# Amandaynzhou/MMT-PSM

Measured on AMD Instinct MI355X. Metric: imgs/sec (student+teacher step, 1000x1000, AUG_K=2), higher is better.
Workload: dtype f32

## Files before the change

include/mmtpsm.h:

```cpp
#ifndef MMTPSM_H
#define MMTPSM_H
#include <stdint.h>
#ifdef __cplusplus
extern "C" {
#endif

#define MMT_EINVAL (-22)

int mmt_version(void);

typedef struct {
  const float* feat[4];
  float* grad_feat[4];
  int H[4];
  int W[4];
  float scale[4];
  int num_levels;
  int N;
  int C;
} mmt_pyramid;

int mmt_roi_align_forward(const mmt_pyramid* pyr , const float* rois, const int32_t* levels,
                          int K, int PH, int PW, int sampling_ratio, float* out, void* stream);
int mmt_roi_align_forward_bf16(const mmt_pyramid* pyr , const float* rois, const int32_t* levels,
// ... 106 lines not shown
  const void* w_src_scale;
  int x_planes_layout;
  void* y_rb;
  long y_rb_stride;
  const float* y_rb_scale;
  void* y_amax_next;
  int x_planes_lag;
  int y_rb_rows;
} mmt_conv_args;

int mmt_conv_forward(const mmt_conv_args* a , void* stream);
int mmt_conv_variant(const mmt_conv_args* a );
int mmt_conv_ksplit(const mmt_conv_args* a );
int mmt_conv_wants_planes(const mmt_conv_args* a );
int mmt_set_conv_precision(int mode);
int mmt_amax(const float* x, long n, const float* rowscale, long inner, int rows, float* amax , void* stream);
int mmt_amax_stats(const float* x, long n, float* slot , void* stream);
int mmt_sum_stats(const float* a, const float* b, const float* c, const float* d, float* y, long n,
                  float* slot , void* stream);
int mmt_stats_combine(const float* const* slots , int n, float* out , void* stream);
int mmt_split_planes_f16(const float* x, void* planes, long plane_stride, long n, float scale, const float* amax ,
                         float* scale_out , float* amax_next ,
                         float* zero_slot , void* stream);
int mmt_pack_weight_f16(const float* w, void* planes, long plane_stride, int Cout, int K, float scale, const float* amax,
                        float* scale_out, void* stream);
int mmt_pack_weight_flipped_f16(const float* w, const float* scale, void* planes, long plane_stride, int Cout, int KH, int KW,
                                int Cin, const float* amax, float* scale_out, void* stream);
int mmt_conv3x3_strip_f16x2(const mmt_conv_args* a , const float* s_x , const float* s_w , void* stream);
int mmt_conv_forward_f16x2(const mmt_conv_args* a , const float* x_amax , const float* s_w , void* stream);
int mmt_get_conv_precision(void);
int mmt_stem_fused(const float* x, int N, int H, int W, const float* w_s2d, const void* w_planes, long w_plane_stride,
                   const float* s_w , const float* scale, const float* shift, const float* x_slot , float* y,
                   float* y_slot , void* stream);
int mmt_conv_wgrad_planes_splits(const mmt_conv_args* a );
int mmt_conv_wgrad_planes(const mmt_conv_args* a , const float* dy, const void* x_planes, long x_plane_stride,
                          const void* dy_planes, long dy_plane_stride, const float* s_x, const float* s_dy, const float* rowscale,
                          float* dw, float* dbias, float* workspace, void* stream);
typedef struct {
  void* fn;
  long a[16];
} mmt_call;
int mmt_replay(const mmt_call* calls , int n, int* failed_index );
int mmt_split_planes_f16_rb(const float* x, void* planes, long plane_stride, int rows, int W, int C, const float* amax,
                            float* scale_out, void* stream);
int mmt_conv_writes_rb(const mmt_conv_args* a );
typedef struct mmt_wgrad_job {
  mmt_conv_args a;
  const float* dy; const float* rowscale; float* dw; float* dbias;
  const void* x_planes; long x_plane_stride; const void* dy_planes; long dy_plane_stride; const float* s_x; const float* s_dy;
} mmt_wgrad_job;
int mmt_conv_wgrad_group_workspace(const mmt_wgrad_job* jobs , int n, long* floats_out );
int mmt_conv_wgrad_group(const mmt_wgrad_job* jobs , int n, float* workspace, long workspace_floats, void* stream);
int mmt_sum_stats_rb(const float* a, const float* b, const float* c, const float* d, float* y, int rows, int W, int C, float* slot,
                     void* planes, long plane_stride, const float* scale, float* amax_next, void* stream);
int mmt_rb_scales_update(float* state, int n, void* stream);
int mmt_conv_forward_pg(const mmt_conv_args* a , const float* s_x , const float* s_w , int tile_rows,
                        int ksplit, void* stream);
int mmt_conv_pg_plan(const mmt_conv_args* a , int* tile_rows, int* ksplit);
int mmt_conv_pg_wanted(const mmt_conv_args* a );
typedef struct { long src_off, dst_off; int Cout, K, unit0, pad; } mmt_pack_desc;
long mmt_packed_weight_elems(int Cout, int K);
int mmt_pack_weight(const float* w, void* planes, long plane_stride, int Cout, int K, void* stream);
int mmt_pack_weight_flipped(const float* w, const float* scale, void* planes, long plane_stride, int Cout, int KH, int KW,
                            int Cin, void* stream);
int mmt_split_planes(const float* x, void* planes, long plane_stride, long n, void* stream);
typedef struct { const float* w; const float* scale; void* dst; long plane_stride; int Cout, KH, KW, Cin, unit0, pad; } mmt_flip_desc;
// ... 72 lines not shown
```

mmt-psm_amd/maskrcnn_benchmark/_hip.py:

```python
import ctypes
import weakref
import os
import threading as _threading

import torch

_HERE = os.path.dirname(os.path.abspath(__file__))
LIB_PATH = os.path.join(os.path.dirname(_HERE), "libmmtpsm.so")

c_void_p, c_int, c_float, c_double, c_int64 = ctypes.c_void_p, ctypes.c_int, ctypes.c_float, ctypes.c_double, ctypes.c_int64


class Pyramid(ctypes.Structure):
    _fields_ = [("feat", c_void_p * 4), ("grad_feat", c_void_p * 4), ("H", c_int * 4), ("W", c_int * 4),
                ("scale", c_float * 4), ("num_levels", c_int), ("N", c_int), ("C", c_int)]


class ConvArgs(ctypes.Structure):
    _fields_ = [("x", c_void_p), ("w", c_void_p), ("scale", c_void_p), ("shift", c_void_p), ("res", c_void_p),
                ("mask", c_void_p), ("mul", c_void_p), ("y", c_void_p),
                ("N", c_int), ("H", c_int), ("W", c_int), ("Cin", c_int), ("Cout", c_int), ("KH", c_int),
                ("KW", c_int), ("stride", c_int), ("pad", c_int), ("Ho", c_int), ("Wo", c_int),
                ("relu", c_int), ("res_mode", c_int), ("out_stride", c_int), ("out_H", c_int), ("out_W", c_int),
                ("mask_scale", c_float), ("w_planes", c_void_p), ("w_plane_stride", ctypes.c_long),
                ("x_planes", c_void_p), ("x_plane_stride", ctypes.c_long),
                ("y_planes", c_void_p), ("y_plane_stride", ctypes.c_long), ("io_bf16", c_int), ("y_amax", c_void_p),
                ("f16_x_amax", c_void_p), ("f16_dy_amax", c_void_p), ("y_amax_stats", c_int),
                ("f16_guard_x", c_void_p), ("f16_guard_dy", c_void_p), ("w_src", c_void_p), ("w_src_scale", c_void_p),
                ("x_planes_layout", c_int),
                ("y_rb", c_void_p), ("y_rb_stride", ctypes.c_long), ("y_rb_scale", c_void_p), ("y_amax_next", c_void_p),
                ("x_planes_lag", c_int), ("y_rb_rows", c_int)]


IO_X, IO_Y, IO_RES, IO_MASK, IO_DY = 1, 2, 4, 8, 16


class WgradJob(ctypes.Structure):
    _fields_ = [("a", ConvArgs), ("dy", c_void_p), ("rowscale", c_void_p), ("dw", c_void_p), ("dbias", c_void_p),
                ("x_planes", c_void_p), ("x_plane_stride", ctypes.c_long), ("dy_planes", c_void_p), ("dy_plane_stride", ctypes.c_long),
                ("s_x", c_void_p), ("s_dy", c_void_p)]


class RpnLevel(ctypes.Structure):
    _fields_ = [("head", c_void_p), ("anchors", c_void_p), ("topk", c_void_p), ("HW", c_int), ("k", c_int),
                ("out_off", c_int), ("pad", c_int)]


class RpnTopkLevel(ctypes.Structure):
    _fields_ = [("head", c_void_p), ("topk", c_void_p), ("HW", c_int), ("k", c_int)]


class RpnSelectArgs(ctypes.Structure):
    _fields_ = [("lv", RpnLevel * 8), ("L", c_int), ("N", c_int), ("A", c_int), ("C", c_int), ("sumk", c_int),
                ("clipv", c_float), ("lim", c_void_p), ("boxes", c_void_p), ("scores", c_void_p), ("idx", c_void_p),
                ("box_reg", c_void_p)]


class RpnPostArgs(ctypes.Structure):
    _fields_ = [("boxes", c_void_p), ("scores", c_void_p), ("idx", c_void_p), ("box_reg", c_void_p), ("keep", c_void_p),
                ("keep_cnt", c_void_p), ("seg_off", c_int * 9), ("own_pre", c_int * 8), ("L", c_int), ("N", c_int),
                ("sumk", c_int), ("kmax", c_int), ("post_n", c_int), ("fpn_post_n", c_int), ("training", c_int),
                ("cap", c_int), ("min_size_filter", c_int), ("pad", c_int), ("gt", c_void_p), ("gt_off", c_void_p),
                ("out_boxes", c_void_p), ("out_scores", c_void_p),
                ("out_idx", c_void_p), ("out_reg", c_void_p), ("out_level", c_void_p), ("out_cnt", c_void_p),
                ("key_scratch", c_void_p)]


# ... 57 lines not shown
                     c_void_p, c_void_p],
    "mmt_box_loss": [c_void_p, c_void_p, c_void_p, c_void_p, c_int, c_int, c_void_p, c_void_p, c_void_p, c_void_p],
    "mmt_box_loss_rows": [c_void_p, c_void_p, c_void_p, c_void_p, c_int, c_int, c_void_p, c_void_p, c_void_p, c_void_p, c_void_p],
    "mmt_relation_attention_fwd": [c_void_p, c_void_p, c_void_p, c_void_p, c_void_p, c_int, c_int, c_int, c_int, c_int, c_int, c_float,
                                   c_void_p, c_void_p, c_void_p],
    "mmt_relation_attention_bwd": [c_void_p, c_void_p, c_void_p, c_void_p, c_void_p, c_void_p, c_int, c_int, c_int, c_int, c_int, c_float,
                                   c_void_p, c_void_p, c_void_p, c_void_p, c_void_p, c_void_p],
    "mmt_ciam_fwd": [c_void_p, c_void_p, c_int, c_int, c_int, c_int, c_void_p, c_void_p, c_void_p, c_void_p, c_void_p],
    "mmt_ciam_bwd": [c_void_p, c_void_p, c_int, c_int, c_int, c_int, c_void_p, c_void_p, c_void_p, c_void_p, c_void_p, c_void_p,
                     c_void_p, c_void_p, c_void_p],
    "mmt_stats_combine": [c_void_p, c_int, c_void_p, c_void_p],
    "mmt_sum_stats": [c_void_p, c_void_p, c_void_p, c_void_p, c_void_p, ctypes.c_long, c_void_p, c_void_p],
    "mmt_split_planes_f16": [c_void_p, c_void_p, ctypes.c_long, ctypes.c_long, c_float, c_void_p, c_void_p, c_void_p, c_void_p, c_void_p],
    "mmt_split_planes_f16_rb": [c_void_p, c_void_p, ctypes.c_long, c_int, c_int, c_int, c_void_p, c_void_p, c_void_p],
    "mmt_replay": [c_void_p, c_int, c_void_p],
    "mmt_conv_writes_rb": [ctypes.POINTER(ConvArgs)],
    "mmt_conv_wgrad_group_workspace": [c_void_p, c_int, ctypes.POINTER(ctypes.c_long)],
    "mmt_conv_wgrad_group": [c_void_p, c_int, c_void_p, ctypes.c_long, c_void_p],
    "mmt_sum_stats_rb": [c_void_p, c_void_p, c_void_p, c_void_p, c_void_p, c_int, c_int, c_int, c_void_p, c_void_p, ctypes.c_long, c_void_p,
                         c_void_p, c_void_p],
    "mmt_rb_scales_update": [c_void_p, c_int, c_void_p],
    "mmt_conv_wgrad_planes_splits": [ctypes.POINTER(ConvArgs)],
    "mmt_conv_wgrad_planes": [ctypes.POINTER(ConvArgs), c_void_p, c_void_p, ctypes.c_long, c_void_p, ctypes.c_long, c_void_p, c_void_p,
                              c_void_p, c_void_p, c_void_p, c_void_p, c_void_p],
    "mmt_pack_weight_f16": [c_void_p, c_void_p, ctypes.c_long, c_int, c_int, c_float, c_void_p, c_void_p, c_void_p],
    "mmt_pack_weight_flipped_f16": [c_void_p, c_void_p, c_void_p, ctypes.c_long, c_int, c_int, c_int, c_int, c_void_p, c_void_p, c_void_p],
    "mmt_conv3x3_strip_f16x2": [ctypes.POINTER(ConvArgs), c_void_p, c_void_p, c_void_p],
    "mmt_conv_forward_f16x2": [ctypes.POINTER(ConvArgs), c_void_p, c_void_p, c_void_p],
    "mmt_conv_forward_pg": [ctypes.POINTER(ConvArgs), c_void_p, c_void_p, c_int, c_int, c_void_p],
    "mmt_conv_pg_plan": [ctypes.POINTER(ConvArgs), c_void_p, c_void_p],
    "mmt_conv_pg_wanted": [ctypes.POINTER(ConvArgs)],
    "mmt_stem_fused": [c_void_p, c_int, c_int, c_int, c_void_p, c_void_p, ctypes.c_long, c_void_p, c_void_p, c_void_p, c_void_p, c_void_p,
                       c_void_p, c_void_p],
    "mmt_maxpool3x3s2_bf16": [c_void_p, c_void_p, c_int, c_int, c_int, c_int, c_int, c_int, c_void_p],
    "mmt_gconv3x3_forward": [c_void_p, c_void_p, c_void_p, c_void_p, c_void_p, c_int, c_int, c_int, c_int, c_int, c_int, c_int, c_void_p],
    "mmt_gconv3x3_dgrad": [c_void_p, c_void_p, c_void_p, c_void_p, c_void_p, c_void_p, c_int, c_int, c_int, c_int, c_int, c_int, c_void_p],
    "mmt_gconv3x3_wgrad": [c_void_p, c_void_p, c_void_p, c_void_p, c_int, c_int, c_int, c_int, c_int, c_int, c_void_p],
    "mmt_mask_bce": [c_void_p, c_void_p, c_void_p, c_int, c_int, c_int, c_float, c_void_p, c_void_p, c_void_p],
    "mmt_mgd_level_forward": [c_void_p, ctypes.POINTER(MgdTeachers), c_void_p, c_int, c_int, c_int, c_int, c_void_p, c_void_p],
    "mmt_mgd_level_backward": [c_void_p, ctypes.POINTER(MgdTeachers), c_void_p, c_int, c_int, c_int, c_int, c_void_p, c_void_p, c_void_p],
    "mmt_mgd_views_forward": [ctypes.POINTER(MgdStudents), ctypes.POINTER(MgdTeachers), c_void_p, c_int, c_int, c_int, c_int, c_void_p,
                              c_void_p],
    "mmt_mgd_views_backward": [ctypes.POINTER(MgdStudents), ctypes.POINTER(MgdTeachers), c_void_p, c_int, c_int, c_int, c_int, c_void_p,
                               c_void_p, c_void_p],
    "mmt_mask_pool": [c_void_p, c_int, c_int, c_int, c_int, c_int, c_void_p, c_void_p],
    "mmt_psm_rows": [c_void_p, c_int, c_void_p, c_int, c_int, c_void_p, c_float, c_int, c_int, c_void_p, c_void_p, c_void_p],
    "mmt_psm_variance": [c_void_p, c_int, c_int, c_int, c_int, c_void_p, c_void_p],
    "mmt_ema_update": [c_void_p, c_void_p, c_int64, c_double, c_void_p],
    "mmt_sgd_momentum": [c_void_p, c_void_p, c_void_p, c_int64, c_float, c_float, c_float, c_int, c_void_p],
    "mmt_paste_masks": [c_void_p, c_void_p, c_void_p, c_void_p, c_int, c_int, c_int, c_int, c_int, c_float, c_void_p, c_void_p],
    "mmt_paste_mask_stack": [c_void_p, c_void_p, c_int, c_int, c_int, c_int, c_float, c_void_p, c_void_p],
    "mmt_polygon_targets": [c_void_p, c_void_p, c_void_p, c_void_p, c_int, c_int, c_void_p, c_void_p, c_void_p],
}

_lib = None
PROFILE = None
PROFILE_ALL = False
_BF16_STORAGE = os.environ.get("MMT_BF16_STORAGE", "0") != "0"


F16X2_DEFAULT = os.environ.get("MMT_F16X2", "1") != "0"
F16X2 = F16X2_DEFAULT
F16X2_TILED = True
F16_STATS = {"wgrad": 0, "conv": 0, "tiled": 0, "pg": 0, "amax_pass": 0, "fallback": 0, "weight_pack": 0}
WGRAD_F16_MIN_ELEMS = 1 << 22
_F16W = {}


def set_f16x2(on):
    global F16X2
    F16X2 = F16X2_DEFAULT if on is None else bool(on)
    _PLAN_EPOCH[0] += 1
    _PLAN.clear()
    _F16W.clear()
    _F16SITE.clear()
    _SITES.clear()
    rb_reset()


STAT_W = 40
_POOL_SLOTS = 2048
F16_CREST_HI, F16_CREST_LO = 2.0 ** 17, 2.0 ** 15


class _StatPool(object):
    __slots__ = ("dev", "host", "event", "next", "gen", "host_gen", "base")

    def __init__(self, device):
        self.dev = torch.zeros((_POOL_SLOTS, STAT_W), dtype=torch.float32, device=device)
        self.host = torch.zeros((_POOL_SLOTS, STAT_W), dtype=torch.float32).pin_memory()
        self.event, self.next, self.gen, self.host_gen = None, 0, 0, -1
        self.base = self.dev.data_ptr()

    def retire(self):
        self.host.copy_(self.dev, non_blocking=True)
        self.event = torch.cuda.Event()
        self.event.record()
# ... 527 lines not shown
    def __del__(self):
        try:
            p = self.pool
            if p is not None:
                self.pool = None
                _POOL_GRAVE.append(p)
        except Exception:
            pass


_POOL_GRAVE = []


def _drain_pools():
    while _POOL_GRAVE:
        try:
            _POOL_GRAVE.pop()
        except IndexError:
            break


def record_torch(fn):
    rec = getattr(_TLS, "rec", None)
    if rec is not None:
        def w(_fn=fn):
            _fn()
            return 0
        rec.calls.append((w, ()))


def planned(tag, fn, x):
    env = os.environ.get
    key = (tag, tuple(x.shape), x.dtype, _stream(), _PLAN_EPOCH[0], PLANES_EPOCH, LAYOUT_EPOCH[0], F16X2, _PREC, _BF16_STORAGE, _RB_EPOCH[0],
           env("MMT_STRIP"), env("MMT_SPLITK"), env("MMT_ROWS"), env("MMT_PG"), env("MMT_C64"), env("MMT_DIRECT_EPI"))
    if getattr(_TLS, "rec", None) is None and _POOL_GRAVE:
        _drain_pools()
    with _LP_LOCK:
        plan = _LAUNCH_PLANS.pop(key, None)
        if plan is None:
            while len(_LAUNCH_PLANS) >= _LP_MAX:
                _LAUNCH_PLANS.pop(next(iter(_LAUNCH_PLANS)))
            plan = LaunchPlan(x.device)
        _LAUNCH_PLANS[key] = plan
    plan.seen += 1
    if plan.seen == 1 or plan.dead or getattr(_TLS, "rec", None) is not None:
        return fn(x)
    if plan.seen == 2:
        _TLS.rec = plan
        try:
            with torch.cuda.use_mem_pool(plan.pool):
                plan.result = fn(x)
        except BaseException:
            with _LP_LOCK:
                _LAUNCH_PLANS.pop(key, None)
            raise
        finally:
            _TLS.rec = None
        plan.in_ptr = x.data_ptr()
        if not any(type(a) is int and a == plan.in_ptr for _f, args in plan.calls for a in args):
            dead_pool, plan.pool = plan.pool, None
            plan.dead, plan.calls = True, []
            del dead_pool
        return plan.result
    plan.slot_buf.zero_()
    old, new = plan.in_ptr, x.data_ptr()
    if C_REPLAY:
        segs = getattr(plan, "segs", None)
# ... 759 lines not shown
    Ho, Wo = _conv_out_hw(H, W, KH, KW, stride, pad)
    a = _conv_shape(ConvArgs(), N, H, W, Cin, Cout, KH, KW, stride, pad, Ho, Wo)
    a.x = x.data_ptr()
    y = empty_nhwc(N, Cout, Ho, Wo, x.device)
    a.y = y.data_ptr()
    a.scale, a.shift, a.relu = _p(scale), _p(shift), 1 if relu else 0
    if res is not None:
        a.res, a.res_mode = nhwc(res).data_ptr(), 1
    if mask is not None:
        a.mask, a.mask_scale = nhwc(mask).data_ptr(), float(mask_scale)
    slot = _amax_slot(x.device)
    a.y_amax, a.y_amax_stats = slot.ptr, 1
    return _conv_f16(a, K_PG, x, src, y, slot, None, int(tile_rows), int(ksplit), xp, None, False)


def stem_fused(x, w_s2d, scale, shift):
    _dev(x)
    N, C, Hh, W = x.shape
    if C != 3 or not x.is_contiguous() or x.dtype != torch.float32 or (Hh & 3) or (W & 3) or tuple(w_s2d.shape) != (64, 16, 4, 4):
        raise RuntimeError("stem_fused: (N, 3, H, W) fp32 NCHW with H, W % 4 == 0 and the 64 x 16 x 4 x 4 space-to-depth filter")
    w = nhwc(w_s2d)
    am = _amax_of(x)
    if type(am[0]) is not _Slot:
        raise RuntimeError("stem_fused: the input needs a full statistics slot")
    wp16, sw = f16_weight_planes(w)
    y = empty_nhwc(N, 64, Hh // 4, W // 4, x.device)
    slot = _amax_slot(x.device)
    _check(lib().mmt_stem_fused(x.data_ptr(), N, Hh, W, w.data_ptr(), wp16.data_ptr(), wp16.stride(0), sw.data_ptr(), _p(scale), _p(shift),
                                am[0].ptr, y.data_ptr(), slot.ptr, _stream()), "mmt_stem_fused")
    y._mmt_amax = (slot, y._version)
    return y


def conv_pg_plan(N, Cin, H, W, Cout, KH, KW, stride, pad):
    Ho, Wo = _conv_out_hw(H, W, KH, KW, stride, pad)
    a = _conv_shape(ConvArgs(), N, H, W, Cin, Cout, KH, KW, stride, pad, Ho, Wo)
    a.x = a.w_planes = 16
    rows, ks = c_int(0), c_int(0)
    _check(lib().mmt_conv_pg_plan(ctypes.byref(a), ctypes.byref(rows), ctypes.byref(ks)), "mmt_conv_pg_plan")
    return rows.value, ks.value


PLANES = {}
GRAD_SLOTS = {}
PLANES_EPOCH = 0


def packed_elems(cout, k):
    return (k // 16) * ((cout + 31) // 32) * 512


def pack_weight(w):
    cout = w.shape[0]
    k = w.numel() // cout
    planes = torch.empty((3, packed_elems(cout, k)), dtype=torch.bfloat16, device=w.device)
    _check(lib().mmt_pack_weight(w.data_ptr(), planes.data_ptr(), planes.stride(0), cout, k, _stream()), "mmt_pack_weight")
    return planes


def pack_weight_flipped(w, scale=None):
    Cout, Cin, KH, KW = w.shape
    if get_conv_precision() == 0 or (Cout & 15) or Cin <= 32:
        return None
    w = nhwc(w)
    ptr, key = w.data_ptr(), None
    ent = PLANES.get(ptr)
# ... 565 lines not shown
```

mmt-psm_amd/maskrcnn_benchmark/layers/fused.py:

```python
import torch

from .. import _hip as H


_NONE = {}


def _none_like(x):
    t = _NONE.get(x.device)
    if t is None:
        t = _NONE[x.device] = torch.empty((0,), dtype=torch.float32, device=x.device)
    return t


def _dst(t):
    return getattr(t, "_flat_grad", None) if t is not None else None


def _touch(*slots):
    for d in slots:
        if d is not None:
            ent = H.GRAD_SLOTS.get(d.data_ptr())
            if ent is not None and ent[0]() is not None:
                ent[0]().touched.add(ent[1])
# ... 177 lines not shown
        gc = g.contiguous()
        g4 = gc.view(R, O, 1, 1)
        _carry_stats(g, gc)
        _carry_stats(gc, g4)
        dx = dw = db = None
        if ctx.needs_input_grad[1]:
            dw, db = _wgrad(x4, g4, w4, 1, 0, None, has_b, *ctx.dst)
            dw = dw.view(O, K) if dw is not None else None
        if ctx.needs_input_grad[0]:
            d4 = _dgrad(g4, w4, x4.shape, 1, 0, None, x4 if input_relu else None, in_mask_scale)
            dx = d4.view(R, K)
            _carry_stats(d4, dx)
        return dx, dw, db, None, None, None, None


def linear(x, w, b=None, relu=False, input_relu=False, in_mask_scale=1.0, mul=None):
    return LinearFn.apply(x, w, b, relu, input_relu, in_mask_scale, mul)


def batch_slice(t, lo, hi):
    v = t[lo:hi]
    H.carry(t, v, images=(lo, hi))
    return v


def _grouped(w2):
    return w2.shape[1] != w2.shape[0]


def _strides(stride, in_3x3):
    return (1, stride) if in_3x3 else (stride, 1)


def bottleneck_forward(x, w1, w2, w3, wd, bn, stride, in_3x3=False):
    s1, b1, s2, b2, s3, b3, sd, bd = bn
    if _grouped(w2):
        if H.bf16_storage():
            raise NotImplementedError("grouped bottlenecks (NUM_GROUPS > 1) are not offered with bf16 activation storage")
        s1x1, s3x3 = _strides(stride, in_3x3)
        o1 = H.conv_forward(x, w1, s1, b1, s1x1, 0, relu=True)
        o2 = H.gconv3x3_forward(o1, w2, s2, b2, s3x3, relu=True)
        r = x if wd is None else H.conv_forward(x, wd, sd, bd, stride, 0)
        out = H.conv_forward(o2, w3, s3, b3, 1, 0, relu=True, res=r, res_mode=1)
        return o1, o2, out
    if in_3x3 and stride != 1:
        raise NotImplementedError("NUM_GROUPS=1 with STRIDE_IN_1X1=False: the dense strided 3x3 data gradient is not built")
    mid = w1.shape[0]
    ho, wo = (x.shape[2] + stride - 1) // stride, (x.shape[3] + stride - 1) // stride
    wp = H.planes_wanted_3x3(x.shape[0], mid, ho, wo, w2.shape[0])
    od = torch.bfloat16 if H.bf16_storage() else None
    o1 = H.conv_forward(x, w1, s1, b1, stride, 0, relu=True, want_planes=wp, out_dtype=od,
                        rb_site=("o1", w2.data_ptr()) if mid >= 128 else None)
    o2 = H.conv_forward(o1, w2, s2, b2, 1, 1, relu=True, out_dtype=od)
    r = x if wd is None else H.conv_forward(x, wd, sd, bd, stride, 0, out_dtype=od)
    out = H.conv_forward(o2, w3, s3, b3, 1, 0, relu=True, res=r, res_mode=1, out_dtype=od)
    return o1, o2, out


class BottleneckFn(torch.autograd.Function):

    @staticmethod
    def forward(ctx, x, w1, w2, w3, wd, bn, stride, pre=None, in_3x3=False):
        s1, b1, s2, b2, s3, b3, sd, bd = bn
        x = H.nhwc(x)
        o1, o2, out = pre if pre is not None else bottleneck_forward(x, w1, w2, w3, wd, bn, stride, in_3x3)
        ctx.in_3x3 = in_3x3
        ctx.save_for_backward(x, o1, o2, w1, w2, w3, wd if wd is not None else _none_like(x))
        ctx.bn = (s1, s2, s3, sd)
        ctx.stride = stride
        ctx.has_ds = wd is not None
        ctx.dst = (_dst(w1), _dst(w2), _dst(w3), _dst(wd))
        return out

    @staticmethod
    def backward(ctx, g):
        x, o1, o2, w1, w2, w3, wd = ctx.saved_tensors
        s1, s2, s3, sd = ctx.bn
        stride = ctx.stride
        g = H.nhwc(g)
        d1, d2, d3, dd = ctx.dst
        if _grouped(w2):
            return BottleneckFn._backward_grouped(ctx, g)
        dw3, _ = _wgrad(o2, g, w3, 1, 0, s3, dst_w=d3)
        d_o2 = _dgrad(g, w3, o2.shape, 1, 0, s3, mask=o2, out_dtype=o2.dtype,
                      want_planes=H.planes_wanted_3x3(o2.shape[0], o2.shape[1], o2.shape[2], o2.shape[3], w2.shape[1]),
                      rb_site=("d_o2", w2.data_ptr()) if o2.shape[1] >= 128 else None)
        dw2, _ = _wgrad(o1, d_o2, w2, 1, 1, s2, dst_w=d2)
        d_o1 = _dgrad(d_o2, w2, o1.shape, 1, 1, s2, mask=o1, out_dtype=o1.dtype)
        dw1, _ = _wgrad(x, d_o1, w1, stride, 0, s1, dst_w=d1)
        dwd = dx = None
        if ctx.has_ds:
            dwd, _ = _wgrad(x, g, wd, stride, 0, sd, dst_w=dd)
        if ctx.needs_input_grad[0]:
            if ctx.has_ds:
                t = _dgrad(d_o1, w1, (x.shape[0], x.shape[1], g.shape[2], g.shape[3]), 1, 0, s1, out_dtype=x.dtype)
                dx = _dgrad(g, wd, x.shape, stride, 0, sd, mask=x, res=t, res_mode=1, out_dtype=x.dtype) if stride > 1 else \
                    _dgrad(g, wd, x.shape, 1, 0, sd, mask=x, res=t, res_mode=1, out_dtype=x.dtype)
            else:
# ... 439 lines not shown
```

Measured before the change: 128.3.

## Fuse frozen 256-64-256 bottleneck into a single f16x2 MFMA kernel

Adds a HIP kernel that runs the whole non-downsampling bottleneck (1x1, 3x3, 1x1 plus residual and ReLU) per 8x16 output tile, keeping the 1x1 output (with halo) and the 3x3 output in LDS as split f16 hi/lo planes instead of writing them to global memory. It is used only when no input needs gradients (e.g. the teacher or frozen stages), stride is 1 and channel counts are 256/64/256. It is meant to remove the intermediate activation round trips and the extra launches. In exchange the 1x1 is recomputed on halo pixels, there is a per-tile scalar fallback path when range checks fail, and LDS use per block is large, which may limit occupancy.

Measured after the change: 129.0 (median of 6 runs). Within noise of the previous version (+0.5%).

```diff
diff --git a/include/mmtpsm.h b/include/mmtpsm.h
--- a/include/mmtpsm.h
+++ b/include/mmtpsm.h
@@ -162,6 +162,18 @@
 int mmt_stem_fused(const float* x, int N, int H, int W, const float* w_s2d, const void* w_planes, long w_plane_stride,
                    const float* s_w , const float* scale, const float* shift, const float* x_slot , float* y,
                    float* y_slot , void* stream);
+typedef struct {
+  const float* x; float* y;
+  const float* w1; const float* w2; const float* w3;
+  const void* w1_planes; const void* w2_planes; const void* w3_planes;
+  long w1_plane_stride, w2_plane_stride, w3_plane_stride;
+  const float* s_w1; const float* s_w2; const float* s_w3;
+  const float* scale1; const float* shift1; const float* scale2; const float* shift2; const float* scale3; const float* shift3;
+  const float* x_slot;
+  float* y_slot;
+  int N, H, W, Cin, Cmid, Cout;
+} mmt_bneck_args;
+int mmt_bottleneck_fused(const mmt_bneck_args* a , void* stream);
 int mmt_conv_wgrad_planes_splits(const mmt_conv_args* a );
 int mmt_conv_wgrad_planes(const mmt_conv_args* a , const float* dy, const void* x_planes, long x_plane_stride,
                           const void* dy_planes, long dy_plane_stride, const float* s_x, const float* s_dy, const float* rowscale,
diff --git a/mmt-psm_amd/csrc/conv_bneck.hip b/mmt-psm_amd/csrc/conv_bneck.hip
--- /dev/null
+++ b/mmt-psm_amd/csrc/conv_bneck.hip
@@ -0,0 +1,448 @@
+#include "conv_shared.h"
+
+namespace {
+
+struct BneckP {
+  const float* x; float* y;
+  const unsigned short* w1pl; const unsigned short* w2pl; const unsigned short* w3pl;
+  long w1s, w2s, w3s;
+  const float* w1; const float* w2; const float* w3;
+  const float* s1; const float* b1; const float* s2; const float* b2; const float* s3; const float* b3;
+  const float* sw1; const float* sw2; const float* sw3;
+  const float* x_slot; unsigned* y_slot;
+  int N, H, W;
+};
+
+constexpr int BK_PW = 18, BK_PIX = 180;
+constexpr int BK_SLAB1 = 192 * 32, BK_PL1 = 4 * BK_SLAB1;
+constexpr int BK_RING = 2 * BK_PL1;
+constexpr int BK_RED = BK_RING - 384;
+constexpr int BK_SLAB2 = 128 * 32, BK_PL2 = 4 * BK_SLAB2;
+constexpr int BK_LDS = BK_RING + 2 * 16384;
+constexpr unsigned BK_OOB = 0x80000000u;
+
+struct Red3 { float mx, sum, cnt; float ws[4], wc[4]; };
+
+__device__ __forceinline__ Red3 block_red3(float mx, float sum, float cnt, float* const red, const int wave, const int lane) {
+#pragma unroll
+  for (int o = 32; o > 0; o >>= 1) {
+    mx = fmaxf(mx, __shfl_xor(mx, o, 64));
+    sum += __shfl_xor(sum, o, 64);
+    cnt += __shfl_xor(cnt, o, 64);
+  }
+  if (lane == 0) { red[wave] = mx; red[4 + wave] = sum; red[8 + wave] = cnt; }
+  __syncthreads();
+  Red3 r;
+  r.mx = fmaxf(fmaxf(red[0], red[1]), fmaxf(red[2], red[3]));
+#pragma unroll
+  for (int w = 0; w < 4; w++) { r.ws[w] = red[4 + w]; r.wc[w] = red[8 + w]; }
+  r.sum = (r.ws[0] + r.ws[1]) + (r.ws[2] + r.ws[3]);
+  r.cnt = (r.wc[0] + r.wc[1]) + (r.wc[2] + r.wc[3]);
+  return r;
+}
+__device__ __forceinline__ bool tile_bad(const Red3& r) {
+  if (!(r.sum == r.sum) || r.mx > 3.0e38f || r.sum > 3.0e38f) return true;
+  bool bad = false;
+#pragma unroll
+  for (int w = 0; w < 4; w++) bad = bad || (r.ws[w] > 0.f && r.mx * r.wc[w] > r.ws[w] * F16_CREST_HI);
+  return bad;
+}
+__device__ __forceinline__ void split1h(const float v, const float s, unsigned short& h, unsigned short& l) {
+  const float r = __builtin_amdgcn_fmed3f(v * s, -65504.f, 65504.f);
+  const _Float16 hh = (_Float16)r;
+  const _Float16 ll = (_Float16)(r - (float)hh);
+  h = __builtin_bit_cast(unsigned short, hh);
+  l = __builtin_bit_cast(unsigned short, ll);
+}
+
+__global__ __launch_bounds__(256, 2) void bneck_fused_kernel(const BneckP p) {
+  extern __shared__ __attribute__((aligned(16))) float lds[];
+  char* const sm = (char*)lds;
+  float* const red = (float*)(sm + BK_RED);
+  const int tid = threadIdx.x, lane = tid & 63;
+  const int wave = __builtin_amdgcn_readfirstlane(tid >> 6);
+  const int lr = lane & 31, kh2 = lane >> 5;
+  const int tiles_x = (p.W + 15) >> 4, tiles_y = (p.H + 7) >> 3;
+  int bid = blockIdx.x;
+  const int tx = bid % tiles_x; bid /= tiles_x;
+  const int ty = bid % tiles_y;
+  const int img = bid / tiles_y;
+  const int oy0 = ty * 8, ox0 = tx * 16;
+  const F16Guard guard = f16_guard_load(p.x_slot);
+  const __amdgpu_buffer_rsrc_t rw1 = __builtin_amdgcn_make_buffer_rsrc((void*)p.w1pl, 0, 0x7ffffff0, 0x00020000);
+  const __amdgpu_buffer_rsrc_t rw2 = __builtin_amdgcn_make_buffer_rsrc((void*)p.w2pl, 0, 0x7ffffff0, 0x00020000);
+  const __amdgpu_buffer_rsrc_t rw3 = __builtin_amdgcn_make_buffer_rsrc((void*)p.w3pl, 0, 0x7ffffff0, 0x00020000);
+  const int xbytes = (int)((long)p.N * p.H * p.W * 1024);
+  const __amdgpu_buffer_rsrc_t rx = __builtin_amdgcn_make_buffer_rsrc((void*)p.x, 0, xbytes, 0x00020000);
+  const __amdgpu_buffer_rsrc_t ry = __builtin_amdgcn_make_buffer_rsrc((void*)p.y, 0, xbytes, 0x00020000);
+  auto copy_chunk = [&](const __amdgpu_buffer_rsrc_t& rs, const long stride, int t, int buf) {
+#pragma unroll
+    for (int i = 0; i < 4; i++) {
+      const int item = wave * 4 + i, st = item >> 2, q = (item >> 1) & 1, blk = item & 1;
+      __builtin_amdgcn_raw_ptr_buffer_load_lds(rs, (lds_ptr_t)(sm + BK_RING + buf * 16384 + ((st * 2 + q) * 2 + blk) * 1024), 16,
+                                               (int)((q * stride + (long)((t * 4 + st) * 2 + blk) * 512 + lane * 8) * 2), 0, 0, 0);
+    }
+  };
+  auto copy_w3 = [&](int it, int buf) {
+#pragma unroll
+    for (int i = 0; i < 4; i++) {
+      const int item = wave * 4 + i, pnl = item >> 3, kt = (item >> 1) & 3, q = item & 1;
+      __builtin_amdgcn_raw_ptr_buffer_load_lds(rw3, (lds_ptr_t)(sm + BK_RING + buf * 16384 + ((pnl * 4 + kt) * 2 + q) * 1024), 16,
+                                               (int)((q * p.w3s + (long)(kt * 8 + 2 * it + pnl) * 512 + lane * 8) * 2), 0, 0, 0);
+    }
+  };
+  const bool x_bad = f16_guard_bad(guard);
+  const float sx = f16_scale_of(guard.amax);
+  const int boff = BK_RING + lr * 32 + (((kh2 ^ (lr >> 3)) & 1) << 4);
+  auto arow = [&](int r) { return 8 * (r >> 2) + (r & 3) + 4 * kh2; };
+
+  f32x16 acc1[2][2];
+#pragma unroll
+  for (int t = 0; t < 2; t++)
+#pragma unroll
+    for (int b = 0; b < 2; b++)
+#pragma unroll
+      for (int r = 0; r < 16; r++) acc1[t][b][r] = 0.f;
+  auto patch_pixel = [&](int P) {
+    const int pr = P / BK_PW, pc = P - pr * BK_PW;
+    const int iy = oy0 - 1 + pr, ix = ox0 - 1 + pc;
+    const bool ok = P < BK_PIX && (unsigned)iy < (unsigned)p.H && (unsigned)ix < (unsigned)p.W;
+    return ok ? (img * p.H + iy) * p.W + ix : -1;
+  };
+  if (!x_bad) {
+    unsigned abase[2];
+#pragma unroll
+    for (int t = 0; t < 2; t++) {
+      const int px = patch_pixel(32 * (wave + 4 * t) + lr);
+      abase[t] = px >= 0 ? ((unsigned)px * 256u + 8u * kh2) * 4u : BK_OOB;
+    }
+    f32x4 ra[2][4][2];
+    auto load_a = [&](int c) {
+#pragma unroll
+      for (int t = 0; t < 2; t++)
+#pragma unroll
+        for (int st = 0; st < 4; st++)
+#pragma unroll
+          for (int h = 0; h < 2; h++)
+            ra[t][st][h] = __builtin_bit_cast(f32x4, __builtin_amdgcn_raw_buffer_load_b128(rx, (int)(abase[t] + (4 * c + st) * 64 + h * 16), 0, 0));
+    };
+    copy_chunk(rw1, p.w1s, 0, 0);
+    load_a(0);
+#pragma unroll
+    for (int c = 0; c < 4; c++) {
+      asm volatile("s_waitcnt vmcnt(0) lgkmcnt(0)" ::: "memory");
+      __syncthreads();
+      uint4 fa[2][4][2];
+#pragma unroll
+      for (int t = 0; t < 2; t++)
+#pragma unroll
+        for (int st = 0; st < 4; st++) {
+          uint2 o0[2], o1[2];
+          split4h(ra[t][st][0], sx, o0);
+          split4h(ra[t][st][1], sx, o1);
+#pragma unroll
+          for (int q = 0; q < 2; q++) fa[t][st][q] = uint4{o0[q].x, o0[q].y, o1[q].x, o1[q].y};
+        }
+      if (c + 1 < 4) {
+        copy_chunk(rw1, p.w1s, c + 1, (c + 1) & 1);
+        load_a(c + 1);
+      }
+      const char* const pb = sm + boff + (c & 1) * 16384;
+#pragma unroll
+      for (int st = 0; st < 4; st++) {
+        f16x8 fb[2][2];
+#pragma unroll
+        for (int q = 0; q < 2; q++)
+#pragma unroll
+          for (int b = 0; b < 2; b++) fb[q][b] = *(const f16x8*)(pb + ((st * 2 + q) * 2 + b) * 1024);
+#pragma unroll
+        for (int t = 0; t < 2; t++)
+#pragma unroll
+          for (int pr = 0; pr < 3; pr++) {
+            const int qa = pr == 1 ? 1 : 0, qb = pr == 0 ? 1 : 0;
+#pragma unroll
+            for (int b = 0; b < 2; b++)
+              acc1[t][b] = __builtin_amdgcn_mfma_f32_32x32x16_f16(__builtin_bit_cast(f16x8, fa[t][st][qa]), fb[qb][b], acc1[t][b], 0, 0, 0);
+          }
+        __builtin_amdgcn_sched_barrier(0);
+      }
+    }
+  } else {
+#pragma unroll
+    for (int t = 0; t < 2; t++) {
+      int off[16];
+#pragma unroll
+      for (int r = 0; r < 16; r++) {
+        const int px = patch_pixel(32 * (wave + 4 * t) + arow(r));
+        off[r] = px >= 0 ? px * 256 : -1;
+      }
+#pragma unroll
+      for (int b = 0; b < 2; b++) {
+        const float* const wr = p.w1 + (b * 32 + lr) * 256;
+#pragma unroll 1
+        for (int k = 0; k < 256; k++) {
+          const float w = wr[k];
+#pragma unroll
+          for (int r = 0; r < 16; r++) acc1[t][b][r] = fmaf(off[r] >= 0 ? p.x[off[r] + k] : 0.f, w, acc1[t][b][r]);
+        }
+      }
+    }
+  }
+  float mx = 0.f, sum = 0.f, cnt = 0.f;
+  {
+    const float inv = x_bad ? 1.f : 1.f / (sx * *p.sw1);
+#pragma unroll
+    for (int t = 0; t < 2; t++)
+#pragma unroll
+      for (int b = 0; b < 2; b++) {
+        const float sc = p.s1[b * 32 + lr] * inv, sh = p.b1[b * 32 + lr];
+#pragma unroll
+        for (int r = 0; r < 16; r++) {
+          const bool ok = patch_pixel(32 * (wave + 4 * t) + arow(r)) >= 0;
+          const float v = ok ? fmaxf(acc1[t][b][r] * sc + sh, 0.f) : 0.f;
+          acc1[t][b][r] = v;
+          mx = fmaxf(mx, v);
+          sum += v;
+          cnt += ok ? 1.f : 0.f;
+        }
+      }
+  }
+  const Red3 r1 = block_red3(mx, sum, cnt, red, wave, lane);
+  const bool bad1 = tile_bad(r1);
+  const float so1 = f16_scale_of(r1.mx);
+  if (!bad1) copy_chunk(rw2, p.w2s, 0, 0);
+#pragma unroll
+  for (int t = 0; t < 2; t++)
+#pragma unroll
+    for (int b = 0; b < 2; b++) {
+      const int ch = b * 32 + lr;
+#pragma unroll
+      for (int r = 0; r < 16; r++) {
+        const int P = 32 * (wave + 4 * t) + arow(r);
+        if (P < BK_PIX) {
+          if (!bad1) {
+            unsigned short h, l;
+            split1h(acc1[t][b][r], so1, h, l);
+            char* const dst = sm + (ch >> 4) * BK_SLAB1 + P * 32 + ((((ch >> 3) ^ (P >> 3)) & 1) << 4) + (ch & 7) * 2;
+            *(unsigned short*)dst = h;
+            *(unsigned short*)(dst + BK_PL1) = l;
+          } else {
+            lds[P * 64 + ch] = acc1[t][b][r];
+          }
+        }
+      }
+    }
+  f32x16 acc[2];
+#pragma unroll
+  for (int b = 0; b < 2; b++)
+#pragma unroll
+    for (int r = 0; r < 16; r++) acc[b][r] = 0.f;
+  if (!bad1) {
+    const int prow = 2 * wave + (lr >> 4), pcol = lr & 15;
+#pragma unroll 1
+    for (int t = 0; t < 9; t++) {
+      asm volatile("s_waitcnt vmcnt(0) lgkmcnt(0)" ::: "memory");
+      __syncthreads();
+      if (t + 1 < 9) copy_chunk(rw2, p.w2s, t + 1, (t + 1) & 1);
+      const int kh = t / 3, kw = t - kh * 3;
+      const int pidx = (prow + kh) * BK_PW + pcol + kw;
+      const char* const pa = sm + pidx * 32 + (((kh2 ^ (pidx >> 3)) & 1) << 4);
+      const char* const pb = sm + boff + (t & 1) * 16384;
+#pragma unroll
+      for (int st = 0; st < 4; st++) {
+        f16x8 fa[2], fb[2][2];
+        fa[0] = *(const f16x8*)(pa + st * BK_SLAB1);
+        fa[1] = *(const f16x8*)(pa + st * BK_SLAB1 + BK_PL1);
+#pragma unroll
+        for (int q = 0; q < 2; q++)
+#pragma unroll
+          for (int b = 0; b < 2; b++) fb[q][b] = *(const f16x8*)(pb + ((st * 2 + q) * 2 + b) * 1024);
+#pragma unroll
+        for (int pr = 0; pr < 3; pr++) {
+          const int qa = pr == 1 ? 1 : 0, qb = pr == 0 ? 1 : 0;
+#pragma unroll
+          for (int b = 0; b < 2; b++) acc[b] = __builtin_amdgcn_mfma_f32_32x32x16_f16(fa[qa], fb[qb][b], acc[b], 0, 0, 0);
+        }
+      }
+    }
+  } else {
+    __syncthreads();
+    int pix0[16];
+#pragma unroll
+    for (int r = 0; r < 16; r++) pix0[r] = ((2 * wave + (arow(r) >> 4)) * BK_PW + (arow(r) & 15)) * 64;
+#pragma unroll
+    for (int b = 0; b < 2; b++) {
+      const float* const wr = p.w2 + (b * 32 + lr) * 576;
+#pragma unroll 1
+      for (int t = 0; t < 9; t++) {
+        const int kh = t / 3, kw = t - kh * 3;
+        const int po = (kh * BK_PW + kw) * 64;
+#pragma unroll 1
+        for (int ci = 0; ci < 64; ci++) {
+          const float w = wr[t * 64 + ci];
+#pragma unroll
+          for (int r = 0; r < 16; r++) acc[b][r] = fmaf(lds[pix0[r] + po + ci], w, acc[b][r]);
+        }
+      }
+    }
+  }
+  bool pok[16];
+  unsigned pixoff[16];
+#pragma unroll
+  for (int r = 0; r < 16; r++) {
+    const int oy = oy0 + 2 * wave + (arow(r) >> 4), ox = ox0 + (arow(r) & 15);
+    pok[r] = oy < p.H && ox < p.W;
+    pixoff[r] = pok[r] ? (unsigned)((img * p.H + oy) * p.W + ox) * 1024u : BK_OOB;
+  }
+  mx = sum = cnt = 0.f;
+  {
+    const float inv = bad1 ? 1.f : 1.f / (so1 * *p.sw2);
+#pragma unroll
+    for (int b = 0; b < 2; b++) {
+      const float sc = p.s2[b * 32 + lr] * inv, sh = p.b2[b * 32 + lr];
+#pragma unroll
+      for (int r = 0; r < 16; r++) {
+        const float v = pok[r] ? fmaxf(acc[b][r] * sc + sh, 0.f) : 0.f;
+        acc[b][r] = v;
+        mx = fmaxf(mx, v);
+        sum += v;
+        cnt += pok[r] ? 1.f : 0.f;
+      }
+    }
+  }
+  const Red3 r2 = block_red3(mx, sum, cnt, red, wave, lane);
+  const bool bad2 = tile_bad(r2);
+  const float so2 = f16_scale_of(r2.mx);
+  if (!bad2) copy_w3(0, 0);
+#pragma unroll
+  for (int b = 0; b < 2; b++) {
+    const int ch = b * 32 + lr;
+#pragma unroll
+    for (int r = 0; r < 16; r++) {
+      const int P = 32 * wave + arow(r);
+      if (!bad2) {
+        unsigned short h, l;
+        split1h(acc[b][r], so2, h, l);
+        char* const dst = sm + (ch >> 4) * BK_SLAB2 + P * 32 + ((((ch >> 3) ^ (P >> 3)) & 1) << 4) + (ch & 7) * 2;
+        *(unsigned short*)dst = h;
+        *(unsigned short*)(dst + BK_PL2) = l;
+      } else {
+        lds[P * 64 + ch] = acc[b][r];
+      }
+    }
+  }
+  asm volatile("s_waitcnt vmcnt(0) lgkmcnt(0)" ::: "memory");
+  __syncthreads();
+  uint4 fa3[4][2];
+  if (!bad2) {
+    const int P = 32 * wave + lr;
+    const char* const pa = sm + P * 32 + (((kh2 ^ (P >> 3)) & 1) << 4);
+#pragma unroll
+    for (int kt = 0; kt < 4; kt++)
+#pragma unroll
+      for (int q = 0; q < 2; q++) fa3[kt][q] = *(const uint4*)(pa + kt * BK_SLAB2 + q * BK_PL2);
+  } else {
+#pragma unroll
+    for (int kt = 0; kt < 4; kt++)
+#pragma unroll
+      for (int q = 0; q < 2; q++) fa3[kt][q] = uint4{0u, 0u, 0u, 0u};
+  }
+  const float inv3 = bad2 ? 1.f : 1.f / (so2 * *p.sw3);
+  float amx = 0.f, asum = 0.f, acnt = 0.f;
+#pragma unroll 1
+  for (int it = 0; it < 4; it++) {
+    if (!bad2 && it + 1 < 4) copy_w3(it + 1, (it + 1) & 1);
+#pragma unroll
+    for (int pnl = 0; pnl < 2; pnl++) {
+      const int ch = (2 * it + pnl) * 32 + lr;
+      float ur[16];
+#pragma unroll
+      for (int r = 0; r < 16; r++)
+        ur[r] = __builtin_bit_cast(float, __builtin_amdgcn_raw_buffer_load_b32(rx, (int)(pixoff[r] + (unsigned)ch * 4u), 0, 0));
+      f32x16 a3;
+#pragma unroll
+      for (int r = 0; r < 16; r++) a3[r] = 0.f;
+      if (!bad2) {
+        const char* const pb = sm + boff + (it & 1) * 16384 + pnl * 8192;
+#pragma unroll
+        for (int kt = 0; kt < 4; kt++) {
+          f16x8 fb[2];
+#pragma unroll
+          for (int q = 0; q < 2; q++) fb[q] = *(const f16x8*)(pb + (kt * 2 + q) * 1024);
+#pragma unroll
+          for (int pr = 0; pr < 3; pr++) {
+            const int qa = pr == 1 ? 1 : 0, qb = pr == 0 ? 1 : 0;
+            a3 = __builtin_amdgcn_mfma_f32_32x32x16_f16(__builtin_bit_cast(f16x8, fa3[kt][qa]), fb[qb], a3, 0, 0, 0);
+          }
+        }
+      } else {
+        const float* const wr = p.w3 + ch * 64;
+#pragma unroll 1
+        for (int k = 0; k < 64; k++) {
+          const float w = wr[k];
+#pragma unroll
+          for (int r = 0; r < 16; r++) a3[r] = fmaf(lds[(32 * wave + arow(r)) * 64 + k], w, a3[r]);
+        }
+      }
+      const float sc = p.s3[ch] * inv3, sh = p.b3[ch];
+#pragma unroll
+      for (int r = 0; r < 16; r++) {
+        float v = a3[r] * sc + sh;
+        v += ur[r];
+        v = fmaxf(v, 0.f);
+        const float av = pok[r] ? fabsf(v) : 0.f;
+        amx = fmaxf(amx, av);
+        asum += av;
+        acnt += pok[r] ? 1.f : 0.f;
+        __builtin_amdgcn_raw_buffer_store_b32(__builtin_bit_cast(unsigned, v), ry, (int)(pixoff[r] + (unsigned)ch * 4u), 0, 0);
+      }
+    }
+    asm volatile("s_waitcnt vmcnt(0) lgkmcnt(0)" ::: "memory");
+    __syncthreads();
+  }
+  if (p.y_slot) {
+    const bool stats = (blockIdx.x & 63) == 0;
+    const Red3 ro = block_red3(amx, asum, acnt, red, wave, lane);
+    if (tid == 0) {
+      const unsigned bits = __builtin_bit_cast(unsigned, ro.mx);
+      if (ro.mx > 0.f && bits > __hip_atomic_load(p.y_slot, __ATOMIC_RELAXED, __HIP_MEMORY_SCOPE_AGENT)) atomicMax(p.y_slot, bits);
+      if (stats && ro.cnt > 0.f) {
+        const int k = (blockIdx.x >> 6) & 15;
+        atomicAdd((float*)p.y_slot + 1 + k, ro.sum);
+        atomicAdd((float*)p.y_slot + 17 + k, ro.cnt);
+      }
+    }
+  }
+}
+
+}
+
+extern "C" int mmt_bottleneck_fused(const mmt_bneck_args* a, void* stream) {
+  if (!a || !a->x || !a->y || !a->w1 || !a->w2 || !a->w3 || !a->w1_planes || !a->w2_planes || !a->w3_planes || !a->s_w1 || !a->s_w2 ||
+      !a->s_w3 || !a->scale1 || !a->shift1 || !a->scale2 || !a->shift2 || !a->scale3 || !a->shift3 || !a->x_slot)
+    return MMT_EINVAL;
+  if (a->N <= 0 || a->H <= 0 || a->W <= 0 || a->Cin != 256 || a->Cmid != 64 || a->Cout != 256 || precision() != 3) return MMT_EINVAL;
+  if (((size_t)a->x & 15) || ((size_t)a->y & 15) || ((size_t)a->w1_planes & 15) || ((size_t)a->w2_planes & 15) || ((size_t)a->w3_planes & 15) ||
+      (a->w1_plane_stride & 7) || (a->w2_plane_stride & 7) || (a->w3_plane_stride & 7))
+    return MMT_EINVAL;
+  if ((long)a->N * a->H * a->W * 1024 >= (1L << 31)) return MMT_EINVAL;
+  BneckP p;
+  p.x = a->x; p.y = a->y;
+  p.w1pl = (const unsigned short*)a->w1_planes; p.w2pl = (const unsigned short*)a->w2_planes; p.w3pl = (const unsigned short*)a->w3_planes;
+  p.w1s = a->w1_plane_stride; p.w2s = a->w2_plane_stride; p.w3s = a->w3_plane_stride;
+  p.w1 = a->w1; p.w2 = a->w2; p.w3 = a->w3;
+  p.s1 = a->scale1; p.b1 = a->shift1; p.s2 = a->scale2; p.b2 = a->shift2; p.s3 = a->scale3; p.b3 = a->shift3;
+  p.sw1 = a->s_w1; p.sw2 = a->s_w2; p.sw3 = a->s_w3;
+  p.x_slot = a->x_slot; p.y_slot = (unsigned*)a->y_slot;
+  p.N = a->N; p.H = a->H; p.W = a->W;
+  static bool done = false;
+  if (!done) {
+    const hipError_t e = hipFuncSetAttribute((const void*)bneck_fused_kernel, hipFuncAttributeMaxDynamicSharedMemorySize, BK_LDS);
+    if (e != hipSuccess) return (int)e;
+    done = true;
+  }
+  const int tiles = a->N * mmt_cdiv(a->H, 8) * mmt_cdiv(a->W, 16);
+  hipLaunchKernelGGL(bneck_fused_kernel, dim3(tiles), dim3(256), BK_LDS, (hipStream_t)stream, p);
+  MMT_LAUNCH_CHECK();
+  return 0;
+}
diff --git a/mmt-psm_amd/maskrcnn_benchmark/_hip.py b/mmt-psm_amd/maskrcnn_benchmark/_hip.py
--- a/mmt-psm_amd/maskrcnn_benchmark/_hip.py
+++ b/mmt-psm_amd/maskrcnn_benchmark/_hip.py
@@ -33,6 +33,16 @@
 
 
 IO_X, IO_Y, IO_RES, IO_MASK, IO_DY = 1, 2, 4, 8, 16
+
+
+class BneckArgs(ctypes.Structure):
+    _fields_ = [("x", c_void_p), ("y", c_void_p), ("w1", c_void_p), ("w2", c_void_p), ("w3", c_void_p),
+                ("w1_planes", c_void_p), ("w2_planes", c_void_p), ("w3_planes", c_void_p),
+                ("w1_plane_stride", ctypes.c_long), ("w2_plane_stride", ctypes.c_long), ("w3_plane_stride", ctypes.c_long),
+                ("s_w1", c_void_p), ("s_w2", c_void_p), ("s_w3", c_void_p),
+                ("scale1", c_void_p), ("shift1", c_void_p), ("scale2", c_void_p), ("shift2", c_void_p),
+                ("scale3", c_void_p), ("shift3", c_void_p), ("x_slot", c_void_p), ("y_slot", c_void_p),
+                ("N", c_int), ("H", c_int), ("W", c_int), ("Cin", c_int), ("Cmid", c_int), ("Cout", c_int)]
 
 
 class WgradJob(ctypes.Structure):
@@ -156,6 +166,7 @@
     "mmt_conv_pg_wanted": [ctypes.POINTER(ConvArgs)],
     "mmt_stem_fused": [c_void_p, c_int, c_int, c_int, c_void_p, c_void_p, ctypes.c_long, c_void_p, c_void_p, c_void_p, c_void_p, c_void_p,
                        c_void_p, c_void_p],
+    "mmt_bottleneck_fused": [ctypes.POINTER(BneckArgs), c_void_p],
     "mmt_maxpool3x3s2_bf16": [c_void_p, c_void_p, c_int, c_int, c_int, c_int, c_int, c_int, c_void_p],
     "mmt_gconv3x3_forward": [c_void_p, c_void_p, c_void_p, c_void_p, c_void_p, c_int, c_int, c_int, c_int, c_int, c_int, c_int, c_void_p],
     "mmt_gconv3x3_dgrad": [c_void_p, c_void_p, c_void_p, c_void_p, c_void_p, c_void_p, c_int, c_int, c_int, c_int, c_int, c_int, c_void_p],
@@ -186,7 +197,7 @@
 F16X2_DEFAULT = os.environ.get("MMT_F16X2", "1") != "0"
 F16X2 = F16X2_DEFAULT
 F16X2_TILED = True
-F16_STATS = {"wgrad": 0, "conv": 0, "tiled": 0, "pg": 0, "amax_pass": 0, "fallback": 0, "weight_pack": 0}
+F16_STATS = {"wgrad": 0, "conv": 0, "tiled": 0, "pg": 0, "amax_pass": 0, "fallback": 0, "weight_pack": 0, "bneck": 0}
 WGRAD_F16_MIN_ELEMS = 1 << 22
 _F16W = {}
 
@@ -780,7 +791,7 @@
 def planned(tag, fn, x):
     env = os.environ.get
     key = (tag, tuple(x.shape), x.dtype, _stream(), _PLAN_EPOCH[0], PLANES_EPOCH, LAYOUT_EPOCH[0], F16X2, _PREC, _BF16_STORAGE, _RB_EPOCH[0],
-           env("MMT_STRIP"), env("MMT_SPLITK"), env("MMT_ROWS"), env("MMT_PG"), env("MMT_C64"), env("MMT_DIRECT_EPI"))
+           env("MMT_STRIP"), env("MMT_SPLITK"), env("MMT_ROWS"), env("MMT_PG"), env("MMT_C64"), env("MMT_DIRECT_EPI"), env("MMT_BNECK_FUSED"))
     if getattr(_TLS, "rec", None) is None and _POOL_GRAVE:
         _drain_pools()
     with _LP_LOCK:
@@ -1606,6 +1617,49 @@
     return y
 
 
+BNECK_FUSED_DEFAULT = "0"
+
+
+def bottleneck_fused_wanted(x, w1, w2, w3):
+    if os.environ.get("MMT_BNECK_FUSED", "1") == "0":
+        return False
+    if not (F16X2 and get_conv_precision() == 3 and not _BF16_STORAGE and x.is_cuda and x.dtype == torch.float32 and w1.dtype == torch.float32):
+        return False
+    if (tuple(w1.shape) != (64, 256, 1, 1) or tuple(w2.shape) != (64, 64, 3, 3) or tuple(w3.shape) != (256, 64, 1, 1)
+            or x.dim() != 4 or x.shape[1] != 256 or x.numel() * 4 >= (1 << 31)):
+        return False
+    am = _recorded(x)
+    if am is None or type(am[0]) is not _Slot:
+        return False
+    return _site_ok((w1.data_ptr(), False), x)
+
+
+def bottleneck_fused(x, w1, w2, w3, bn):
+    _dev(x)
+    x = nhwc(x)
+    N, C, Hh, W = x.shape
+    am = _recorded(x)
+    a = BneckArgs()
+    keep = []
+    for i, w in enumerate((w1, w2, w3), 1):
+        w = nhwc(w)
+        pl, sw = f16_weight_planes(w)
+        keep.append((w, pl, sw))
+        setattr(a, "w%d" % i, w.data_ptr())
+        setattr(a, "w%d_planes" % i, pl.data_ptr())
+        setattr(a, "w%d_plane_stride" % i, pl.stride(0))
+        setattr(a, "s_w%d" % i, sw.data_ptr())
+    a.scale1, a.shift1, a.scale2, a.shift2, a.scale3, a.shift3 = (_p(t) for t in bn[:6])
+    y = empty_nhwc(N, 256, Hh, W, x.device)
+    slot = _amax_slot(x.device)
+    a.x, a.y, a.x_slot, a.y_slot = x.data_ptr(), y.data_ptr(), am[0].ptr, slot.ptr
+    a.N, a.H, a.W, a.Cin, a.Cmid, a.Cout = N, Hh, W, 256, 64, 256
+    F16_STATS["bneck"] += 1
+    _check(lib().mmt_bottleneck_fused(ctypes.byref(a), _stream()), "mmt_bottleneck_fused")
+    y._mmt_amax = (slot, y._version)
+    return y
+
+
 def conv_pg_plan(N, Cin, H, W, Cout, KH, KW, stride, pad):
     Ho, Wo = _conv_out_hw(H, W, KH, KW, stride, pad)
     a = _conv_shape(ConvArgs(), N, H, W, Cin, Cout, KH, KW, stride, pad, Ho, Wo)
diff --git a/mmt-psm_amd/maskrcnn_benchmark/layers/fused.py b/mmt-psm_amd/maskrcnn_benchmark/layers/fused.py
--- a/mmt-psm_amd/maskrcnn_benchmark/layers/fused.py
+++ b/mmt-psm_amd/maskrcnn_benchmark/layers/fused.py
@@ -233,8 +233,11 @@
     return (1, stride) if in_3x3 else (stride, 1)
 
 
-def bottleneck_forward(x, w1, w2, w3, wd, bn, stride, in_3x3=False):
+def bottleneck_forward(x, w1, w2, w3, wd, bn, stride, in_3x3=False, frozen=False):
     s1, b1, s2, b2, s3, b3, sd, bd = bn
+    if (frozen and wd is None and stride == 1 and not w1.requires_grad and not _grouped(w2)
+            and H.bottleneck_fused_wanted(x, w1, w2, w3)):
+        return None, None, H.bottleneck_fused(x, w1, w2, w3, bn)
     if _grouped(w2):
         if H.bf16_storage():
             raise NotImplementedError("grouped bottlenecks (NUM_GROUPS > 1) are not offered with bf16 activation storage")
@@ -264,7 +267,10 @@
     def forward(ctx, x, w1, w2, w3, wd, bn, stride, pre=None, in_3x3=False):
         s1, b1, s2, b2, s3, b3, sd, bd = bn
         x = H.nhwc(x)
-        o1, o2, out = pre if pre is not None else bottleneck_forward(x, w1, w2, w3, wd, bn, stride, in_3x3)
+        frozen = pre is None and not any(ctx.needs_input_grad)
+        o1, o2, out = pre if pre is not None else bottleneck_forward(x, w1, w2, w3, wd, bn, stride, in_3x3, frozen)
+        if o1 is None:
+            return out
         ctx.in_3x3 = in_3x3
         ctx.save_for_backward(x, o1, o2, w1, w2, w3, wd if wd is not None else _none_like(x))
         ctx.bn = (s1, s2, s3, sd)
```
